# StanfordASL/pmpc

Measured on AMD Instinct MI355X. Metric: SCP iterations/sec (M particles x N horizon), higher is better.
Workload: dtype f64; 1 GPU; quadrotor x12 u4 M=4096 N=50 Nc=1 box-u, full SCP iteration (on-device linearise + c_lqp_solve-equivalent + residual), BASELINE config D; timed window = SCP iterations 6..2477 from the cold start X_prev = x0, U_prev = U_ref (the active-set round count falls as the SCP loop converges, so the rate depends on the window); particles_per_gpu=4096, parallelism=particle-shard x1, scp_loop=library (pmpc_scp_loop_device), ipm_warm_start=True

## Files before the change

include/pmpc_abi.h:

```cpp
#ifndef PMPC_ABI_H
#define PMPC_ABI_H

#include <stddef.h>

#ifdef __cplusplus
extern "C" {
#endif


void c_lqp_solve(double *X_out, double *U_out, size_t xdim, size_t udim, size_t N, size_t M, long long Nc,
                 double *x0, double *f, double *fx, double *fu, double *X_prev, double *U_prev, double *Q,
                 double *R, double *X_ref, double *U_ref, double *lx, double *ux, double *lu, double *uu,
                 double reg_x, double reg_u, double *slew_reg, double *slew_reg0, double *slew_um1,
                 long long verbose);

void c_lcone_solve(double *X_out, double *U_out, size_t xdim, size_t udim, size_t N, size_t M, long long Nc,
                   double *x0, double *f, double *fx, double *fu, double *X_prev, double *U_prev, double *Q,
                   double *R, double *X_ref, double *U_ref, double *lx, double *ux, double *lu, double *uu,
                   double reg_x, double reg_u, double *slew_reg, double *slew_reg0, double *slew_um1,
                   long long verbose, double smooth_alpha, char *solver);

void pmpc_lqp_solve_host(double *X_out, double *U_out, size_t xdim, size_t udim, size_t N, size_t M, long long Nc,
                         double *x0, double *f, double *fx, double *fu, double *X_prev, double *U_prev, double *Q,
                         double *R, double *X_ref, double *U_ref, double *lx, double *ux, double *lu, double *uu,
// ... 80 lines not shown
int pmpc_comm_unique_id(void *unique_id_128);
int pmpc_comm_init(pmpc_ctx *ctx, int rank, int world, const void *unique_id_128);
int pmpc_comm_init_mock(pmpc_ctx *ctx, int rank, int world, int group);
int pmpc_comm_rank(pmpc_ctx *ctx);
int pmpc_comm_world(pmpc_ctx *ctx);

int pmpc_linearize_device(pmpc_ctx *ctx, int model, size_t N, size_t M, const double *x0, const double *X_prev,
                          const double *U_prev, const double *params, double *f, double *fx, double *fu);

int pmpc_linearize_device_f32(pmpc_ctx *ctx, int model, size_t N, size_t M, const double *x0, const double *X_prev,
                              const double *U_prev, const double *params, double *f, float *fx, float *fu);

int pmpc_rollout_device(pmpc_ctx *ctx, int model, size_t N, size_t M, const double *x0, const double *U, const double *params, double *X);

int pmpc_shift_plan_device(pmpc_ctx *ctx, int model, size_t N, size_t M, size_t s, const double *X, const double *U,
                           const double *params, const double *U_tail, double *X_new, double *U_new, double *um1_new);

int pmpc_shift_active_set_device(pmpc_ctx *ctx, size_t N, size_t M, size_t udim, long long Nc, size_t s, const double *U,
                                 const double *U_tail, const int *act, const double *lo, const double *hi, double *U_new, int *act_new);

int pmpc_warm_shift_device(pmpc_ctx *ctx, size_t N, size_t M, size_t udim, long long Nc, size_t s, const double *U, const double *U_tail,
                           const double *lo, const double *hi, double *U_new, int *shifted);

int pmpc_warm_set_read_device(pmpc_ctx *ctx, int *act_out, size_t n);

int pmpc_linearize_compact_device(pmpc_ctx *ctx, int model, size_t N, size_t M, const double *x0, const double *X_prev,
                                  const double *U_prev, const double *params, double *f, double *jc);
int pmpc_expand_jac_device(pmpc_ctx *ctx, int model, size_t N, size_t M, const double *jc, double *fx, double *fu, int orient);
long long pmpc_jac_compact_doubles(int model, size_t N, size_t M);
int pmpc_jac_live_mask(int model, unsigned char *fx_mask, unsigned char *fu_mask);

int pmpc_as_sweep_variant(int sweep, int xdim, int udim, int M, int Nc, unsigned flags, const int *knobs, int *out);

int pmpc_as_sweep_launches(int sweep, unsigned long long *out, int n, int reset);
void pmpc_as_sweep_knobs(int *out);

int pmpc_scp_residual_device(pmpc_ctx *ctx, size_t xdim, size_t udim, size_t N, size_t M, const double *X, const double *X_prev,
                             const double *U, const double *U_prev, double *out);

int pmpc_scp_loop_device(pmpc_ctx *ctx, int model, const double *params, const pmpc_problem *p, double *f2, double *fx2, double *fu2,
                         int steps, int first_cold, double *res, pmpc_info *infos, int *last_in_out);

int pmpc_ref_shift_device(pmpc_ctx *ctx, size_t dim, size_t rows, const double *A, const double *c, const double *ref, double *out);
long long pmpc_ref_shift_bad_pivots(pmpc_ctx *ctx, int reset);

typedef struct pmpc_scp_cost {
  int kind;
  int K, pos_dim;
  int pos_idx[3];
  int per_stage;
  const double *centres, *sigma, *w;
} pmpc_scp_cost;
size_t pmpc_abi_scp_cost_size(void);

int pmpc_obstacle_cost_grad_device(pmpc_ctx *ctx, const pmpc_scp_cost *cost, size_t xdim, size_t N, size_t M, const double *X_prev,
                                   double *cx);
int pmpc_obstacle_ref_shift_device(pmpc_ctx *ctx, const pmpc_scp_cost *cost, size_t xdim, size_t N, size_t M, const double *X_prev,
                                   const double *Q, const double *X_ref, double *out);

int pmpc_scp_loop_device_cost(pmpc_ctx *ctx, int model, const double *params, const pmpc_problem *p, double *f2, double *fx2,
                              double *fu2, int steps, int first_cold, double *res, pmpc_info *infos, int *last_in_out,
                              const pmpc_scp_cost *cost);

typedef struct pmpc_scp_cstr {
  int kind;
  int K, pos_dim;
// ... 40 lines not shown
```

pmpc_amd/_lib.py:

```python
from __future__ import annotations

import ctypes
import os
from pathlib import Path

import numpy as np

_HERE = Path(__file__).resolve().parent
LIB_PATH = Path(os.environ["PMPC_HIP_LIB"]) if os.environ.get("PMPC_HIP_LIB") else _HERE / "libpmpc_hip.so"
_lib = None

c_dp = ctypes.POINTER(ctypes.c_double)

HAS_XBOUNDS, HAS_UBOUNDS, HAS_SLEW, HAS_SLEW0, FORCE_GENERIC, SYMMETRIC_COST, COLD_START, STATIC_CONS_BOUNDS, PREV_IS_LAST_SOLUTION, F32_MATRICES, CONE_OBJECTIVE = 1, 2, 4, 8, 16, 32, 64, 128, 256, 512, 1024

ABI_SYMBOLS = [
    "c_lqp_solve", "c_lcone_solve", "pmpc_lqp_solve_host", "pmpc_lcone_solve_host", "pmpc_create", "pmpc_destroy", "pmpc_stream", "pmpc_sync", "pmpc_lqp_solve_device",
    "pmpc_comm_unique_id", "pmpc_comm_init", "pmpc_comm_rank", "pmpc_comm_world", "pmpc_linearize_device",
    "pmpc_profile_enable", "pmpc_profile_read", "pmpc_version", "pmpc_lcone_solve_device", "pmpc_particle_costs_device", "pmpc_lsoc_solve_device", "pmpc_comm_init_mock",
    "pmpc_scp_residual_device", "pmpc_profile_read_partial", "pmpc_profile_read_all", "pmpc_scp_loop_device", "pmpc_linearize_device_f32",
    "pmpc_set_option", "pmpc_get_option", "pmpc_abi_struct_sizes", "pmpc_lcone_solve_host_ex", "pmpc_restart_stats",
    "pmpc_linearize_compact_device", "pmpc_expand_jac_device", "pmpc_jac_compact_doubles", "pmpc_jac_live_mask",
    "pmpc_as_sweep_variant", "pmpc_as_sweep_launches", "pmpc_as_sweep_knobs",
    "pmpc_ref_shift_device", "pmpc_ref_shift_bad_pivots", "pmpc_obstacle_cost_grad_device", "pmpc_obstacle_ref_shift_device",
    "pmpc_scp_loop_device_cost", "pmpc_abi_scp_cost_size",
    "pmpc_rollout_device", "pmpc_shift_plan_device",
    "pmpc_keepout_augment_device", "pmpc_abi_scp_cstr_size",
    "pmpc_keepout_strip_residual_device", "pmpc_scp_loop_device_cstr", "pmpc_abi_scp_aug_size", "pmpc_scp_loop_follow_ups",
    "pmpc_shift_active_set_device", "pmpc_warm_shift_device", "pmpc_warm_set_read_device",
]


class PmpcProblem(ctypes.Structure):
    _fields_ = (
        [(k, ctypes.c_size_t) for k in ("xdim", "udim", "N", "M")]
        + [("Nc", ctypes.c_longlong), ("flags", ctypes.c_uint), ("reg_x", ctypes.c_double), ("reg_u", ctypes.c_double)]
        + [(k, ctypes.c_void_p) for k in ("x0", "f", "fx", "fu", "X_prev", "U_prev", "Q", "R", "X_ref", "U_ref",
                                          "lx", "ux", "lu", "uu", "slew_reg", "slew_reg0", "slew_um1", "X_out", "U_out", "weights")]
        + [("barrier_mu", ctypes.c_double), ("soc_q", ctypes.c_size_t), ("soc_W", ctypes.c_void_p), ("soc_w0", ctypes.c_void_p),
           ("soc_v", ctypes.c_void_p), ("soc_v0", ctypes.c_double), ("soc_u_interior", ctypes.c_void_p),
           ("cone_count", ctypes.c_size_t), ("cone_sizes", ctypes.POINTER(ctypes.c_int)), ("cone_A", ctypes.c_void_p), ("cone_c", ctypes.c_void_p),
           ("cone_per_stage", ctypes.c_int), ("cone_k", ctypes.c_longlong), ("smooth_cstr", ctypes.c_int), ("smooth_beta", ctypes.c_double)]
    )


class PmpcInfo(ctypes.Structure):
    _fields_ = [("status", ctypes.c_int), ("ipm_iters", ctypes.c_int), ("structured_solves", ctypes.c_int),
                ("fast_path", ctypes.c_int), ("mu", ctypes.c_double), ("slack_res", ctypes.c_double),
                ("max_violation", ctypes.c_double), ("outer_solves", ctypes.c_int), ("active_set_rounds", ctypes.c_int)]


class PmpcScpCost(ctypes.Structure):
    _fields_ = [("kind", ctypes.c_int), ("K", ctypes.c_int), ("pos_dim", ctypes.c_int), ("pos_idx", ctypes.c_int * 3), ("per_stage", ctypes.c_int),
                ("centres", ctypes.c_void_p), ("sigma", ctypes.c_void_p), ("w", ctypes.c_void_p)]


# ... 50 lines not shown
    lib.pmpc_particle_costs_device.argtypes = [vp, ctypes.POINTER(PmpcProblem), vp, vp, vp]
    lib.pmpc_particle_costs_device.restype = ctypes.c_int
    lib.pmpc_comm_unique_id.argtypes = [vp]
    lib.pmpc_comm_unique_id.restype = ctypes.c_int
    lib.pmpc_comm_init.argtypes = [vp, ctypes.c_int, ctypes.c_int, vp]
    lib.pmpc_comm_init.restype = ctypes.c_int
    lib.pmpc_comm_init_mock.argtypes = [vp, ctypes.c_int, ctypes.c_int, ctypes.c_int]
    lib.pmpc_comm_init_mock.restype = ctypes.c_int
    lib.pmpc_comm_rank.argtypes = [vp]
    lib.pmpc_comm_rank.restype = ctypes.c_int
    lib.pmpc_comm_world.argtypes = [vp]
    lib.pmpc_comm_world.restype = ctypes.c_int
    lib.pmpc_linearize_device.argtypes = [vp, ctypes.c_int, sz, sz] + [vp] * 7
    lib.pmpc_linearize_device.restype = ctypes.c_int
    lib.pmpc_linearize_device_f32.argtypes = [vp, ctypes.c_int, sz, sz] + [vp] * 7
    lib.pmpc_linearize_device_f32.restype = ctypes.c_int
    if hasattr(lib, "pmpc_jac_live_mask"):
        lib.pmpc_linearize_compact_device.argtypes = [vp, ctypes.c_int, sz, sz] + [vp] * 6
        lib.pmpc_linearize_compact_device.restype = ctypes.c_int
        lib.pmpc_expand_jac_device.argtypes = [vp, ctypes.c_int, sz, sz, vp, vp, vp, ctypes.c_int]
        lib.pmpc_expand_jac_device.restype = ctypes.c_int
        lib.pmpc_jac_compact_doubles.argtypes = [ctypes.c_int, sz, sz]
        lib.pmpc_jac_compact_doubles.restype = ctypes.c_longlong
        lib.pmpc_jac_live_mask.argtypes = [ctypes.c_int, vp, vp]
        lib.pmpc_jac_live_mask.restype = ctypes.c_int
    if hasattr(lib, "pmpc_as_sweep_variant"):
        lib.pmpc_as_sweep_variant.argtypes = [ctypes.c_int] * 5 + [ctypes.c_uint, ctypes.POINTER(ctypes.c_int), ctypes.POINTER(ctypes.c_int)]
        lib.pmpc_as_sweep_variant.restype = ctypes.c_int
    if hasattr(lib, "pmpc_as_sweep_launches"):
        lib.pmpc_as_sweep_launches.argtypes = [ctypes.c_int, ctypes.POINTER(ctypes.c_ulonglong), ctypes.c_int, ctypes.c_int]
        lib.pmpc_as_sweep_launches.restype = ctypes.c_int
        lib.pmpc_as_sweep_knobs.argtypes = [ctypes.POINTER(ctypes.c_int)]
        lib.pmpc_as_sweep_knobs.restype = None
    lib.pmpc_scp_residual_device.argtypes = [vp, sz, sz, sz, sz] + [vp] * 5
    lib.pmpc_scp_residual_device.restype = ctypes.c_int
    lib.pmpc_profile_enable.argtypes = [vp, ctypes.c_int]
    lib.pmpc_profile_enable.restype = None
    lib.pmpc_profile_read.argtypes = [vp, c_dp, ctypes.POINTER(ctypes.c_longlong)]
    lib.pmpc_profile_read.restype = None
    lib.pmpc_profile_read_partial.argtypes = [vp, ctypes.POINTER(ctypes.c_double), ctypes.POINTER(ctypes.c_longlong)]
    lib.pmpc_profile_read_partial.restype = None
    lib.pmpc_restart_stats.argtypes = [vp, ctypes.POINTER(ctypes.c_ulonglong), ctypes.c_int]
    lib.pmpc_restart_stats.restype = None
    lib.pmpc_profile_read_all.argtypes = [vp, c_dp, ctypes.POINTER(ctypes.c_longlong), ctypes.c_int]
    lib.pmpc_profile_read_all.restype = None
    lib.pmpc_scp_loop_device.argtypes = [vp, ctypes.c_int, vp, ctypes.POINTER(PmpcProblem), vp, vp, vp, ctypes.c_int, ctypes.c_int, vp,
                                         ctypes.POINTER(PmpcInfo), ctypes.POINTER(ctypes.c_int)]
    lib.pmpc_scp_loop_device.restype = ctypes.c_int
    if hasattr(lib, "pmpc_scp_loop_device_cost"):
        lib.pmpc_ref_shift_device.argtypes = [vp, sz, sz, vp, vp, vp, vp]
        lib.pmpc_ref_shift_device.restype = ctypes.c_int
        lib.pmpc_ref_shift_bad_pivots.argtypes = [vp, ctypes.c_int]
        lib.pmpc_ref_shift_bad_pivots.restype = ctypes.c_longlong
        lib.pmpc_obstacle_cost_grad_device.argtypes = [vp, ctypes.POINTER(PmpcScpCost), sz, sz, sz, vp, vp]
        lib.pmpc_obstacle_cost_grad_device.restype = ctypes.c_int
        lib.pmpc_obstacle_ref_shift_device.argtypes = [vp, ctypes.POINTER(PmpcScpCost), sz, sz, sz, vp, vp, vp, vp]
        lib.pmpc_obstacle_ref_shift_device.restype = ctypes.c_int
        lib.pmpc_scp_loop_device_cost.argtypes = lib.pmpc_scp_loop_device.argtypes + [ctypes.POINTER(PmpcScpCost)]
        lib.pmpc_scp_loop_device_cost.restype = ctypes.c_int
        lib.pmpc_abi_scp_cost_size.argtypes = []
        lib.pmpc_abi_scp_cost_size.restype = sz
        if lib.pmpc_abi_scp_cost_size() != ctypes.sizeof(PmpcScpCost):
            raise ImportError(f"{LIB_PATH} and pmpc_amd/_lib.py disagree on pmpc_scp_cost: library {lib.pmpc_abi_scp_cost_size()} bytes, "
                              f"binding {ctypes.sizeof(PmpcScpCost)}: rebuild the library")
    if hasattr(lib, "pmpc_shift_plan_device"):
        lib.pmpc_rollout_device.argtypes = [vp, ctypes.c_int, sz, sz, vp, vp, vp, vp]
# ... 36 lines not shown
    sp, si = sz(0), sz(0)
    lib.pmpc_abi_struct_sizes(ctypes.byref(sp), ctypes.byref(si))
    if (sp.value, si.value) != (ctypes.sizeof(PmpcProblem), ctypes.sizeof(PmpcInfo)):
        raise ImportError(f"{LIB_PATH} ({lib.pmpc_version().decode()}) and pmpc_amd/_lib.py disagree on the ABI structs: library "
                          f"{sp.value}/{si.value} bytes, binding {ctypes.sizeof(PmpcProblem)}/{ctypes.sizeof(PmpcInfo)}: rebuild the library")
    _lib = lib
    return lib


def jac_live_mask(model: int, x: int, u: int):
    lib = load()
    mx, mu = np.zeros(x * x, dtype=np.uint8), np.zeros(x * u, dtype=np.uint8)
    got = lib.pmpc_jac_live_mask(int(model), mx.ctypes.data, mu.ctypes.data)
    if got < 0:
        raise ValueError(f"model {model} is not a built-in model")
    if got != 100 * x + u:
        raise ValueError(f"model {model}: compact records are for dims {got // 100} x {got % 100}, not {x} x {u}")
    return mx.reshape(x, x).T.astype(bool), mu.reshape(u, x).T.astype(bool)


AS_SWEEP_FLAGS = ("defect", "as_settled_in", "mat32", "cone_H", "xb_D", "as_uraw", "as_T")


def as_sweep_variant(sweep: str, x: int, u: int, M: int, Nc: int, flags: int, knobs=None):
    lib = load()
    out = (ctypes.c_int * 8)()
    kn = (ctypes.c_int * 3)(*knobs) if knobs is not None else None
    got = lib.pmpc_as_sweep_variant({"bwd": 0, "fwd": 1}[sweep], x, u, M, Nc, flags, kn, out)
    if got < 0:
        raise ValueError(f"({x}, {u}) is not a compiled pair of the active-set sweeps")
    return tuple(out[:5]), bool(got), tuple(bool(v) for v in out[5:8])


def as_sweep_code(sweep: str, variant) -> int:
    a, b, c, d, e = (int(v) for v in variant)
    if sweep == "bwd":
        return a + 3 * (b + 2 * (c + 2 * (d + 3 * e)))
    return a + 2 * b + 4 * c + 8 * d + 16 * e


def as_sweep_launches(sweep: str, reset: bool = False):
    lib = load()
    sw = {"bwd": 0, "fwd": 1}[sweep]
    n = lib.pmpc_as_sweep_launches(sw, None, 0, 0)
    out = (ctypes.c_ulonglong * n)()
    lib.pmpc_as_sweep_launches(sw, out, n, int(reset))
    return [int(v) for v in out]


def scp_loop_follow_ups(reset: bool = False):
    out = (ctypes.c_ulonglong * 2)()
    load().pmpc_scp_loop_follow_ups(out, int(reset))
    return int(out[0]), int(out[1])


def as_sweep_knobs():
    out = (ctypes.c_int * 3)()
    load().pmpc_as_sweep_knobs(out)
    return tuple(out)


def dptr(a: np.ndarray):
    assert a.dtype == np.float64 and a.flags["C_CONTIGUOUS"]
    return a.ctypes.data_as(c_dp)
```

pmpc_amd/csrc/fast_common.h:

```cpp
#pragma once
#include "pmpc_dev.h"

namespace {

typedef double v4d __attribute__((ext_vector_type(4)));

__device__ __forceinline__ v4d mfma(double a, double b, v4d c) {
  return __builtin_amdgcn_mfma_f64_16x16x4f64(a, b, c, 0, 0, 0);
}
__device__ __forceinline__ double readlane_d(double v, int l) {
  int lo = __builtin_amdgcn_readlane(__double2loint(v), l);
  int hi = __builtin_amdgcn_readlane(__double2hiint(v), l);
  return __hiloint2double(hi, lo);
}
__device__ __forceinline__ double rfl_d(double v) {
  int lo = __builtin_amdgcn_readfirstlane(__double2loint(v));
  int hi = __builtin_amdgcn_readfirstlane(__double2hiint(v));
  return __hiloint2double(hi, lo);
}
template <int CTRL>
__device__ __forceinline__ double dpp_d(double v) {
  int lo = __builtin_amdgcn_mov_dpp(__double2loint(v), CTRL, 0xF, 0xF, true);
  int hi = __builtin_amdgcn_mov_dpp(__double2hiint(v), CTRL, 0xF, 0xF, true);
  return __hiloint2double(hi, lo);
}
__device__ __forceinline__ double row_allsum(double v) {
  v += dpp_d<0xB1>(v);
  v += dpp_d<0x4E>(v);
  v += dpp_d<0x141>(v);
  v += dpp_d<0x140>(v);
  return v;
}
__device__ __forceinline__ void swap32_d(double v, double &a, double &b) {
  auto lo = __builtin_amdgcn_permlane32_swap(__double2loint(v), __double2loint(v), false, false);
  auto hi = __builtin_amdgcn_permlane32_swap(__double2hiint(v), __double2hiint(v), false, false);
  a = __hiloint2double(hi[0], lo[0]);
  b = __hiloint2double(hi[1], lo[1]);
}
__device__ __forceinline__ void swap16_d(double v, double &a, double &b) {
  auto lo = __builtin_amdgcn_permlane16_swap(__double2loint(v), __double2loint(v), false, false);
  auto hi = __builtin_amdgcn_permlane16_swap(__double2hiint(v), __double2hiint(v), false, false);
  a = __hiloint2double(hi[0], lo[0]);
  b = __hiloint2double(hi[1], lo[1]);
}
__device__ __forceinline__ double grp_allsum(double v) {
  double a, b;
  swap32_d(v, a, b);
  v = a + b;
  swap16_d(v, a, b);
  return a + b;
}
__device__ __forceinline__ void grp_gather(double v, double (&out)[4]) {
  double p01, p23;
  swap32_d(v, p01, p23);
  swap16_d(p01, out[0], out[1]);
  swap16_d(p23, out[2], out[3]);
}
__device__ __forceinline__ double rsqrt_d(double d) {
  const double r = __builtin_amdgcn_rsq(d);
  const double e = fma(-0.5 * d * r, r, 0.5);
  return fma(r, e, r);
}
__device__ __forceinline__ const double *badd(const double *p, long long bytes) {
  return (const double *)((const char *)p + bytes);
// ... 103 lines not shown
```

pmpc_amd/csrc/kernels_as.hip:

```cpp
#include <atomic>
#include <type_traits>

#include "fast_common.h"
#include "as_ctl_dev.h"
#include "as_variant.h"
#include "../../include/pmpc_abi.h"
#include "jac_compact.h"

#ifdef PMPC_STAGE_TIMELINE
#define PMPC_TL_STAMPS 10
__device__ unsigned long long pmpc_tl[3][128][PMPC_TL_STAMPS];
#define TL_DECL(kind) unsigned long long tl_[PMPC_TL_STAMPS] = {}; const int tl_kind = (kind); const bool tl_on = blockIdx.x == gridDim.x / 2
#define TL(k) do { __builtin_amdgcn_sched_barrier(0); tl_[k] = __builtin_amdgcn_s_memtime(); __builtin_amdgcn_sched_barrier(0); } while (0)
#define TL_FLUSH(j) do { if (tl_on && threadIdx.x == 0 && (j) < 128) { for (int k_ = 0; k_ < PMPC_TL_STAMPS; k_++) pmpc_tl[tl_kind][j][k_] = tl_[k_]; } } while (0)
#else
#define TL_DECL(kind)
#define TL(k)
#define TL_FLUSH(j)
#endif

#ifndef PMPC_AS_LEAN_WAVES
#define PMPC_AS_LEAN_WAVES 4
#endif
#ifndef PMPC_AS_DEEP_WAVES
#define PMPC_AS_DEEP_WAVES 3
#endif
#ifndef PMPC_AS_DEEP2_MAXM
#define PMPC_AS_DEEP2_MAXM 1024
#endif

namespace {

template <int XD, int UD, int MODE, bool SKIP, bool DEFECT, int EX = 0, class MT = double>
__global__ void __launch_bounds__(64, MODE == 2 ? 2 : (MODE == 1 ? PMPC_AS_DEEP_WAVES : PMPC_AS_LEAN_WAVES)) k_bwd_as(LQArgs a) {
  constexpr bool CONE = EX == 1, XBOX = EX == 2;
  typedef Lane<XD, UD> LT;
  constexpr int KS = LT::KS, XP = LT::XP;
  constexpr bool PADX = (XD != XP);
  constexpr long long D8 = sizeof(double);
  constexpr bool DEEP = MODE != 0, SCHOL = !DEEP;
  constexpr long long MB = sizeof(MT);
  if (a.done && *a.done) return;
  const int lane = threadIdx.x;
  const int N = a.N, Nc = a.Nc, i = a.as_perm ? __builtin_amdgcn_readfirstlane(a.as_perm[blockIdx.x]) : (int)blockIdx.x;
  if (SKIP && a.as_settled_in[i]) {
    const int nc = Nc * UD;
    if (lane < nc) {
      const double *H = a.Hc_part + (size_t)i * nc * nc;
      double acc = 0.0;
      for (int cc = 0; cc < nc; cc++) acc = fma(H[(lane < cc ? lane : cc) + nc * (lane < cc ? cc : lane)], a.as_delta[cc], acc);
      a.gc_part[(size_t)i * nc + lane] += acc;
    }
    return;
  }
  const LT L(lane);
  const int g = L.g, c = L.c;
  const size_t pbase = (size_t)i * N;
  const bool own0 = (i == 0 && a.owner);
  const bool gu = g < UD;
  const double *Z = a.zeros;
  const double pwt = a.pw ? a.pw[i] : 1.0;
  const double regx = pwt * a.reg_x, regu = pwt * a.reg_u;
  const double *Xb = DEFECT ? a.X_prev : a.Xb, *Ub = DEFECT ? a.U_prev : a.Ub;
  constexpr int CKS = 64 * KS + 32;
  int jtop = N - 1, ck_k = 0;
  if (SKIP && a.as_ck) {
    const int jh = a.as_jhi[i];
// ... 5 lines not shown
      atomicAdd(a.ck_stat + (ck_k ? 1 : 3), (unsigned long long)(jtop + 1));
    }
  }
  const double *ck_ = a.as_ck ? ubase(a.as_ck, (long long)i * a.ck_slots * (long long)(CKS * sizeof(double))) : nullptr;

  const bool fF = L.cxv || L.cu;
  const MT *pF = L.cxv ? (const MT *)a.fx + (pbase + jtop) * (XD * XD) + XD * L.oc + L.row0
                       : (L.cu ? (const MT *)a.fu + (pbase + jtop) * (XD * UD) + XD * L.cb + L.row0 : (const MT *)Z);
  int sF = fF ? -(int)MB * (L.cxv ? XD * XD : XD * UD) : 0;
  typedef typename jacc::SpecFor<XD, UD>::list JSpecs;
  if constexpr (JSpecs::COUNT > 0 && std::is_same<MT, double>::value) {
    if (a.jac_compact) {
      const jacc::LaneSel js = jacc::select(JSpecs{}, a.jac_compact, lane);
      const int m = js.bwd;
      if (m != jacc::NONE) {
        pF = m >= 0 ? (const MT *)a.fx + (pbase + jtop) * js.rec + m : (const MT *)a.fx + (size_t)a.M * N * js.rec + (size_t)i * js.pool + (-1 - m);
        sF = m >= 0 ? -(int)MB * js.rec : 0;
      }
    }
  }
  const unsigned lQ = (unsigned)((L.cxv ? XD * L.oc + L.row0 : 0) * MB);
  const double pwt_x = L.cxv ? pwt : 0.0;
  const bool fR = L.cu && gu;
  const unsigned lR = (unsigned)((fR ? g + UD * L.cb : 0) * MB), lRd = (unsigned)((fR ? g + UD * L.cb : 0) * D8);
  const unsigned lxr = (unsigned)(L.row0 * D8), lxc = (unsigned)((L.cxv ? L.oc : 0) * D8);
  const unsigned lug = (unsigned)((gu ? g : 0) * D8);
  const double regx_c = L.cxv ? regx : 0.0;
  const bool umask = L.cu && g == L.cb;
  const double umask_d = umask ? 1.0 : 0.0;
  const bool diag_x = L.cxv && ((c & 3) == g);
  bool dmask[KS];
#pragma unroll
  for (int r = 0; r < KS; r++) dmask[r] = diag_x && (c >> 2) == r;
  const long long px = (long long)(pbase * XD) * D8, pu = (long long)(pbase * UD) * D8;
  const double *Xb_ = ubase(Xb, px), *Xr_ = ubase(a.X_ref, px), *Xp_ = ubase(a.X_prev, px), *f_ = ubase(a.f, px);
  const double *kff_ = ubase(a.kff, pu);
  const void *Q_ = ubase_v(a.Q, (long long)(pbase * (XD * XD)) * MB), *R_ = ubase_v(a.R, (long long)(pbase * (UD * UD)) * MB);
  const void *K_ = ubase_v(a.K, (long long)(pbase * 64) * MB);
  auto xoff = [&](int jj) { return (long long)(jj * (int)(XD * D8)); };
  auto uoff = [&](int jj) { return (long long)(jj * (int)(UD * D8)); };
  auto ld_Q = [&](int jj, double *dst) {
    const void *q = ubase_v(Q_, (long long)(jj * (int)(XD * XD * MB)));
#pragma unroll
    for (int r = 0; r < KS; r++) {
      const bool rv = !PADX || (L.row0 + r < XD);
      const double v = ldom<MT>(q, rv ? lQ + r * (unsigned)MB : 0u);
      dst[r] = rv ? v : 0.0;
    }
  };
  auto ld_xm = [&](int jj, double *dst) {
    const double *xb = ubase(Xb_, xoff(jj)), *xr = ubase(Xr_, xoff(jj));
#pragma unroll
    for (int r = 0; r < KS; r++) {
      const bool rv = !PADX || (L.row0 + r < XD);
      const unsigned o = rv ? lxr + r * 8u : 0u;
      const double v = pwt * (ldo(xb, o) - ldo(xr, o));
      dst[r] = rv ? v : 0.0;
    }
  };
  auto ld_gx = [&](int jj) -> double {
    if (DEFECT) return 0.0;
    return regx_c * (ldo(ubase(Xb_, xoff(jj)), lxc) - ldo(ubase(Xp_, xoff(jj)), lxc));
  };
  const char *pC = (const char *)Z;
  int sC = 0;
  if (gu && c == XP) { pC = (const char *)(Ub + (pbase + jtop) * UD + g); sC = -UD * (int)D8; }
// ... 104 lines not shown
    for (int r = 0; r < KS; r++) Fr[r] = (!MAIN && j == 0 && L.cxv) ? 0.0 : cur.F[r];
    const double Rc = cur.R;
    const double um_g = pwt * (dpp_d<0x00>(cur.ctl) - dpp_d<0x55>(cur.ctl));
    const int act_g = __builtin_amdgcn_mov_dpp(__double2loint(cur.ctl), 0xAA, 0xF, 0xF, true);
    Du_c = (umask && act_g) ? a.as_big : 0.0;
    const double gu_c0 = DEFECT ? 0.0 : regu_s * dpp_d<0x140>(cur.ctl);
    const bool cone_here = CONE && (MAIN || !cons || own0);
    double gu_c = gu_c0;
    if constexpr (CONE) gu_c = fma(dpp_d<0xFF>(cur.ctl), cone_here ? umask_d : 0.0, gu_c0);
    double Hcone = 0.0;
    if constexpr (CONE) Hcone = cone_here ? cur.ch : 0.0;
    const double df_c = (DEFECT && L.cxv) ? cur.f - xb_carry : 0.0;
    if (DEFECT) xb_carry = cur.xb;
    gx_c = DEFECT ? 0.0 : regx_c * (cur.xb - cur.xp);
    if constexpr (XBOX) gx_c += cur.xg;
    col_to_row<KS>(pwt_x * (cur.xb - cur.xr), g, xm_row);
#pragma unroll
    for (int r = 0; r < KS; r++) Qc[r] = cur.Q[r];
    auto late_pf = [&]() { if (below) fetch_late(j - 1, j >= 2 ? j - 2 : 0, nxt); };
    TL(1);
    if (MODE == 1) late_pf();
    if (MODE != 2 && below) fetch_early(j - 1, nxt);
    TL(2);

    if (DEFECT) {
#pragma unroll
      for (int r = 0; r < KS; r++) s_row[r] += row_allsum(S[r] * df_c);
    }
    double hp = fma(Rc, um_g, gu_c);
#pragma unroll
    for (int r = 0; r < KS; r++) hp = fma(Fr[r], s_row[r], hp);
    const double h_col = grp_allsum(hp);
    double hu[UD];
#pragma unroll
    for (int b = 0; b < UD; b++) hu[b] = readlane_d(h_col, XP + b);

    TL(3);
    v4d H = {0.0, 0.0, 0.0, 0.0};
    double p2q = 0.0;
    if (below) {
#pragma unroll
      for (int r = 0; r < KS; r++) {
        if constexpr (XBOX) H[r] = fma(pwt_x, Qc[r], dmask[r] ? regx + cur.xd : 0.0);
        else H[r] = fma(pwt_x, Qc[r], dmask[r] ? regx : 0.0);
        p2q = fma(Qc[r], xm_row[r], p2q);
      }
    }
    if constexpr (CONE) H[KS] = fma(pwt, Rc, (umask ? regu : 0.0) + (cons ? 0.0 : Du_c + Hcone));
    else H[KS] = fma(pwt, Rc, (umask ? regu : 0.0) + (cons ? 0.0 : Du_c));
    v4d G = {0.0, 0.0, 0.0, 0.0};
#pragma unroll
    for (int r = 0; r < KS; r++) G = mfma(S[r], Fr[r], G);
#pragma unroll
    for (int r = 0; r < KS; r++) H = mfma(Fr[r], G[r], H);

    if (!DEEP && !MAIN) late_pf();
    if (!MAIN && cons) {
      double v = H[KS];
      if (own0) v += CONE ? Du_c + Hcone : Du_c;
      const int nc = Nc * UD;
      if (L.cu && gu) a.Hc_part[(size_t)i * nc * nc + (size_t)(j * UD + g) + (size_t)nc * (j * UD + L.cb)] = v;
      st_rec(j, (L.cxv && gu) ? H[KS] : 0.0);
#pragma unroll
      for (int r = 0; r < KS; r++) S[r] = H[r];
      if (lane < UD) a.gc_part[(size_t)i * (Nc * UD) + j * UD + lane] = pick<UD>(hu, lane);
      if (j == 0) return;
      const double p2 = grp_allsum(p2q);
      s_col = L.cxv ? h_col + p2 + gx_c : 0.0;
      col_to_row<KS>(s_col, g, s_row);
      return;
    }

    TL(4);
    double Lc[UD][UD], Ld[UD], col[UD];
#pragma unroll
    for (int q = 0; q < UD; q++) {
#pragma unroll
      for (int pp = q; pp < UD; pp++) {
        double v = readlane_d(H[KS], (XP + q) + 16 * pp);
#pragma unroll
        for (int k = 0; k < q; k++) v -= Lc[pp][k] * Lc[q][k];
        if (pp == q) {
          bad |= !(v > 0.0);
          Ld[q] = SCHOL ? rfl_d(rsqrt_d(v)) : rsqrt_d(v);
        } else {
          Lc[pp][q] = SCHOL ? rfl_d(v * Ld[q]) : v * Ld[q];
        }
      }
    }
    TL(5);
    double rows4[4];
    grp_gather(H[KS], rows4);
#pragma unroll
    for (int k = 0; k < UD; k++) col[k] = L.cu ? (L.cb == k ? 1.0 : 0.0) : rows4[k];
    chol_solve<UD>(Lc, Ld, col);
    const double Kg = pick<UD>(col, g);
    const double rec = frec ? Kg : 0.0;
    TL(6);
    v4d Sn = mfma(H[KS], (L.cxv && gu) ? -Kg : 0.0, H);
#pragma unroll
    for (int r = 0; r < KS; r++) S[r] = Sn[r];
    st_rec(j, rec);
    if (!DEEP && MAIN) {
      __builtin_amdgcn_sched_barrier(0);
      late_pf();
    }
    const double Kreg = L.cxv ? rec : 0.0;
    const double hug = pick<UD>(hu, g);
    double kq = L.cu ? rec * pick<UD>(hu, L.cb) : 0.0;
    kq += dpp_d<0xB1>(kq);
    kq += dpp_d<0x4E>(kq);
    if (c == XP && gu) gsto(ubase(kff_, uoff(j)), lug, kq);
    TL(7);
    if (!MAIN && j == 0) { TL_FLUSH(j); return; }
    const double red2 = grp_allsum(fma(-Kreg, hug, p2q));
    s_col = L.cxv ? h_col + red2 + gx_c : 0.0;
    col_to_row<KS>(s_col, g, s_row);
    TL(8);
    TL_FLUSH(j);
  };

  const int jmin = Nc > 1 ? Nc : 1;
  int j = jtop;
  if (MODE == 2) {
    Pipe P0, P1, P2;
    auto fetch = [&](int jj, Pipe &q) {
      const int k = jj > 0 ? jj : 0;
      fetch_early(k, q);
      fetch_late(k, k >= 1 ? k - 1 : 0, q);
    };
    fetch(jtop, P0);
    fetch(jtop - 1, P1);
    for (; j - 2 >= jmin; j -= 3) {
      fetch(j - 2, P2);
      stage(std::true_type{}, j, P0, P0);
      __builtin_amdgcn_sched_barrier(0);
      fetch(j - 3, P0);
      stage(std::true_type{}, j - 1, P1, P1);
      __builtin_amdgcn_sched_barrier(0);
      fetch(j - 4, P1);
      stage(std::true_type{}, j - 2, P2, P2);
      __builtin_amdgcn_sched_barrier(0);
    }
    for (; j >= 0; j--) {
      fetch(j - 2, P2);
      if (j >= jmin) stage(std::true_type{}, j, P0, P0);
      else stage(std::false_type{}, j, P0, P0);
      P0 = P1;
      P1 = P2;
    }
  } else {
    Pipe A, B;
    fetch_early(jtop, A);
    fetch_late(jtop, jtop >= 1 ? jtop - 1 : 0, A);
    for (; j >= jmin; j--) {
      stage(std::true_type{}, j, A, B);
      A = B;
    }
    if (j >= jmin) {
      stage(std::true_type{}, j, A, B);
      A = B;
      j--;
    }
    for (; j >= 0; j--) {
      stage(std::false_type{}, j, A, B);
      A = B;
    }
  }
  if (bad && lane == 0) *a.fail = 2;
}

template <int XD, int UD, bool DEFECT, bool PF2, bool CONE = false, class MT = double, bool SENS = false>
__global__ void __launch_bounds__(64, 4) k_fwd_as(LQArgs a) {
  typedef Lane<XD, UD> LT;
  constexpr int KS = LT::KS;
  constexpr bool PADX = (XD != LT::XP);
  constexpr long long D8 = sizeof(double);
  if (a.done && *a.done) return;
  const int lane = threadIdx.x;
  const LT L(lane);
  const int N = a.N, Nc = a.Nc, i = a.as_perm ? __builtin_amdgcn_readfirstlane(a.as_perm[blockIdx.x]) : (int)blockIdx.x, g = L.g, c = L.c;
  const size_t pbase = (size_t)i * N;
  const bool gu = g < UD;
  const double *Z = a.zeros;
  constexpr int MB = (int)sizeof(MT);
  const char *pA = (const char *)Z, *pB = (const char *)Z;
  int sAr = 0, sAj = 0, sBj = 0;
// ... 212 lines not shown
    pS += UD * (int)D8;
    if (store_u) gsto_i(ubase(act_, uoff(j) >> 1), lug >> 1, anew);
    TL(4);
    D[KS] = 0.0;
    double bop = (c < 4 && gu) ? du_q : 0.0;
    if (SENS) {
      const bool sc = c >= 4 && c < 4 + UD && gu;
      const double bs = (!MAIN && j < Nc) ? ((g == c - 4) ? 1.0 : 0.0) : -raw;
      bop = sc ? bs : bop;
    }
    D = mfma(cur.T[KS], bop, D);
    if (SENS) {
      if (c >= 4 && c < 4 + UD) {
        typedef double v2dd __attribute__((ext_vector_type(2)));
        const v2dd lo2 = {D[0], KS > 1 ? D[KS > 1 ? 1 : 0] : 0.0}, hi2 = {KS > 2 ? D[KS > 2 ? 2 : 0] : 0.0, gu ? bop : 0.0};
        __attribute__((address_space(1))) char *t = (__attribute__((address_space(1))) char *)(unsigned long long)ubase(T_, (long long)(j * (int)(64 * D8))) + lT;
        *(v2dd __attribute__((address_space(1))) *)t = lo2;
        *(v2dd __attribute__((address_space(1))) *)(t + 16) = hi2;
      }
    }
    if (DEFECT) {
      const double dfo = own_x ? cur.f - cur.xb : 0.0;
      D[0] += dpp_d<0x00>(dfo);
      if (KS > 1) D[1] += dpp_d<0x55>(dfo);
      if (KS > 2) D[2] += dpp_d<0xAA>(dfo);
    }
    if (own_x) {
      double mine = D[0];
#pragma unroll
      for (int r = 1; r < KS; r++) mine = (c == r) ? D[r] : mine;
      gsto(ubase(Xo_, xoff(j)), lx1, cur.xb + mine);
    }
#pragma unroll
    for (int r = 0; r < KS; r++) V[r] = (c < (SENS ? 4 + UD : 4)) ? D[r] : 0.0;
    TL(5);
    TL_FLUSH(j);
  };

  int nrel_e = 0, nadd_e = 0, nbad_e = 0, jh_e = -1;
  auto settled_update = [&](int j0) {
    double dl[UD];
#pragma unroll
    for (int k = 0; k < UD; k++) dl[k] = readlane_d(dcap, 16 * k);
    const int s16 = lane & 15, q4 = lane >> 4, gs = s16 >> 2, rs = s16 & 3;
    const bool is_x = rs < KS && KS * gs + rs < XD, is_u = rs == 3 && gs < UD;
    const size_t xo = (size_t)(is_x ? KS * gs + rs : 0), uo = (size_t)(is_u ? gs : 0);
    constexpr int SB = 4;
    for (int j4 = j0; j4 < N; j4 += 4 * SB) {
      double dv[SB], xv[SB], ub[SB], kf[SB], lo[SB], hi[SB];
      int act[SB];
#pragma unroll
      for (int q = 0; q < SB; q++) {
        const int jj = j4 + 4 * q + q4, jc = jj < N ? jj : N - 1;
        const double *t = a.as_T + (pbase + jc) * 64 + s16;
        double acc = 0.0;
#pragma unroll
        for (int k = 0; k < UD; k++) acc = fma(gld(t + 16 * k), dl[k], acc);
        dv[q] = acc;
        xv[q] = is_x ? gld(Xb + (pbase + jc) * XD + xo) : 0.0;
        const size_t e = (pbase + jc) * UD + uo;
        ub[q] = is_u ? gld(Ub + e) : 0.0;
        kf[q] = is_u ? gld(a.kff + e) : 0.0;
        lo[q] = is_u ? gld(a.as_lo + e) : 0.0;
        hi[q] = is_u ? gld(a.as_hi + e) : 0.0;
        act[q] = is_u ? a.as_act[e] : 0;
      }
#pragma unroll
// ... 177 lines not shown
  if (!launched) no_such_variant("forward sweep of an active-set round", XD, UD);
}

}

#ifdef PMPC_STAGE_TIMELINE
extern "C" int pmpc_debug_timeline_read(unsigned long long *out) {
  return (int)hipMemcpyFromSymbol(out, HIP_SYMBOL(pmpc_tl), sizeof(unsigned long long) * 3 * 128 * PMPC_TL_STAMPS);
}
#endif
static bool as_dims_compiled(int x, int u) {
#define X(xd, ud) if (x == xd && u == ud) return true;
  PMPC_FAST_DIMS(X)
#undef X
  return false;
}
bool f32_as_dims_supported(int x, int u) { return as_dims_compiled(x, u) && as_f32_dims(x, u); }
bool xbox_as_dims_supported(int x, int u) { return as_dims_compiled(x, u) && as_xbox_dims(x, u); }
bool cone_as_dims_supported(int x, int u) { return as_dims_compiled(x, u) && as_cone_dims(x, u); }
int pmpc_as_sweep_variant(int sweep, int xdim, int udim, int M, int Nc, unsigned flags, const int *knobs, int *out) {
  if ((sweep != 0 && sweep != 1) || !as_dims_compiled(xdim, udim) || !out) return -1;
  const AsSweepKnobs k = knobs ? AsSweepKnobs{knobs[0], knobs[1], knobs[2]} : AsSweepKnobs{PMPC_AS_DEEP2_MAXM, PMPC_AS_DEEP_WAVES * 1024, 1 << 30};
  const bool defect = flags & 1, settled_in = flags & 2, mat32 = flags & 4, cone_H = flags & 8, xb_D = flags & 16, as_uraw = flags & 32, as_T = flags & 64;
  out[5] = f32_as_dims_supported(xdim, udim); out[6] = cone_as_dims_supported(xdim, udim); out[7] = xbox_as_dims_supported(xdim, udim);
  if (sweep == 0) {
    const BwdAsVariant v = select_bwd_as(M, defect, settled_in, mat32, cone_H, xb_D, k);
    out[0] = v.mode; out[1] = v.skip; out[2] = v.defect; out[3] = v.ex; out[4] = v.f32;
    return bwd_as_compiled(v, xdim, udim);
  }
  const FwdAsVariant v = select_fwd_as(M, Nc, defect, mat32, as_uraw, as_T, k);
  out[0] = v.defect; out[1] = v.pf2; out[2] = v.cone; out[3] = v.f32; out[4] = v.sens;
  return fwd_as_compiled(v, xdim, udim);
}
int pmpc_as_sweep_launches(int sweep, unsigned long long *out, int n, int reset) {
  if (sweep != 0 && sweep != 1) return -1;
  std::atomic<unsigned long long> *t = sweep == 0 ? as_bwd_launches : as_fwd_launches;
  const int codes = sweep == 0 ? AS_BWD_CODES : AS_FWD_CODES;
  for (int c = 0; c < codes; c++) {
    const unsigned long long v = reset ? t[c].exchange(0, std::memory_order_relaxed) : t[c].load(std::memory_order_relaxed);
    if (out && c < n) out[c] = v;
  }
  return codes;
}
void pmpc_as_sweep_knobs(int *out) {
  const AsSweepKnobs &k = as_sweep_knobs();
  out[0] = k.deep2_maxm; out[1] = k.deep_maxm; out[2] = k.fwd_pf2_maxm;
}
void launch_bwd_as(const LQArgs &a, hipStream_t s) {
#define X(xd, ud) if (a.x == xd && a.u == ud) { launch_bwd_as_t<xd, ud>(a, s); return; }
  PMPC_FAST_DIMS(X)
#undef X
  no_such_variant("factor sweep of an active-set round", a.x, a.u);
}
void launch_fwd_as(const LQArgs &a, hipStream_t s) {
#define X(xd, ud) if (a.x == xd && a.u == ud) { launch_fwd_as_t<xd, ud>(a, s); return; }
  PMPC_FAST_DIMS(X)
#undef X
  no_such_variant("forward sweep of an active-set round", a.x, a.u);
}
void launch_as_ctl(AsCtl *ctl, const int *cnt_part, int M, const int *fail, int reduce, int decide, int last_of_batch, AsCtl *mirror,
                   unsigned long long *mirror_seq, unsigned long long seq, hipStream_t s, double *tail, const double *viol, const int *open_part) {
  hipLaunchKernelGGL(k_as_ctl, dim3(1), dim3(1024), 0, s, ctl, cnt_part, M, fail, reduce, decide, last_of_batch, mirror, mirror_seq, seq, tail, viol,
                     open_part);
}
void launch_as_perm(const int *settled, int M, int *perm, const int *done, hipStream_t s) {
  hipLaunchKernelGGL(k_as_perm, dim3(1), dim3(1024), 0, s, settled, M, perm, done);
// ... 5 lines not shown
```

Before: 3017 SCP iterations/s.

## Tighten backward active-set sweep registers to fit four waves for x12u4

```diff
diff --git a/include/pmpc_abi.h b/include/pmpc_abi.h
--- a/include/pmpc_abi.h
+++ b/include/pmpc_abi.h
@@ -136,6 +136,8 @@
 
 int pmpc_as_sweep_variant(int sweep, int xdim, int udim, int M, int Nc, unsigned flags, const int *knobs, int *out);
 
+int pmpc_as_sweep_resources(int sweep, int xdim, int udim, const int *variant, int *out);
+
 int pmpc_as_sweep_launches(int sweep, unsigned long long *out, int n, int reset);
 void pmpc_as_sweep_knobs(int *out);
 
diff --git a/pmpc_amd/_lib.py b/pmpc_amd/_lib.py
--- a/pmpc_amd/_lib.py
+++ b/pmpc_amd/_lib.py
@@ -21,7 +21,7 @@
     "pmpc_scp_residual_device", "pmpc_profile_read_partial", "pmpc_profile_read_all", "pmpc_scp_loop_device", "pmpc_linearize_device_f32",
     "pmpc_set_option", "pmpc_get_option", "pmpc_abi_struct_sizes", "pmpc_lcone_solve_host_ex", "pmpc_restart_stats",
     "pmpc_linearize_compact_device", "pmpc_expand_jac_device", "pmpc_jac_compact_doubles", "pmpc_jac_live_mask",
-    "pmpc_as_sweep_variant", "pmpc_as_sweep_launches", "pmpc_as_sweep_knobs",
+    "pmpc_as_sweep_variant", "pmpc_as_sweep_launches", "pmpc_as_sweep_knobs", "pmpc_as_sweep_resources",
     "pmpc_ref_shift_device", "pmpc_ref_shift_bad_pivots", "pmpc_obstacle_cost_grad_device", "pmpc_obstacle_ref_shift_device",
     "pmpc_scp_loop_device_cost", "pmpc_abi_scp_cost_size",
     "pmpc_rollout_device", "pmpc_shift_plan_device",
@@ -138,6 +138,9 @@
         lib.pmpc_as_sweep_launches.restype = ctypes.c_int
         lib.pmpc_as_sweep_knobs.argtypes = [ctypes.POINTER(ctypes.c_int)]
         lib.pmpc_as_sweep_knobs.restype = None
+    if hasattr(lib, "pmpc_as_sweep_resources"):
+        lib.pmpc_as_sweep_resources.argtypes = [ctypes.c_int] * 3 + [ctypes.POINTER(ctypes.c_int), ctypes.POINTER(ctypes.c_int)]
+        lib.pmpc_as_sweep_resources.restype = ctypes.c_int
     lib.pmpc_scp_residual_device.argtypes = [vp, sz, sz, sz, sz] + [vp] * 5
     lib.pmpc_scp_residual_device.restype = ctypes.c_int
     lib.pmpc_profile_enable.argtypes = [vp, ctypes.c_int]
@@ -240,6 +243,18 @@
     return tuple(out[:5]), bool(got), tuple(bool(v) for v in out[5:8])
 
 
+def as_sweep_resources(sweep: str, x: int, u: int, variant):
+    out = (ctypes.c_int * 4)()
+    got = load().pmpc_as_sweep_resources({"bwd": 0, "fwd": 1}[sweep], x, u, (ctypes.c_int * 5)(*(int(v) for v in variant)), out)
+    if got == -2:
+        return None
+    if got == -1:
+        raise ValueError(f"({x}, {u}) is not a compiled pair of the active-set sweeps")
+    if got != 0:
+        raise RuntimeError(f"pmpc_as_sweep_resources: HIP error {got}")
+    return dict(zip(("regs", "scratch_bytes", "lds_bytes", "max_threads"), (int(v) for v in out)))
+
+
 def as_sweep_code(sweep: str, variant) -> int:
     a, b, c, d, e = (int(v) for v in variant)
     if sweep == "bwd":
diff --git a/pmpc_amd/csrc/fast_common.h b/pmpc_amd/csrc/fast_common.h
--- a/pmpc_amd/csrc/fast_common.h
+++ b/pmpc_amd/csrc/fast_common.h
@@ -30,6 +30,15 @@
   v += dpp_d<0x141>(v);
   v += dpp_d<0x140>(v);
   return v;
+}
+template <int C0, int NB>
+__device__ __forceinline__ double row_own_bcast(double v) {
+  static_assert(NB >= 1 && NB <= 4 && C0 >= 0 && C0 + NB <= 16, "row_own_bcast: lanes C0 .. C0 + NB - 1 of a 16-lane row");
+  double o = NB == 4 ? __builtin_amdgcn_update_dpp(0.0, v, 0x150 + C0, 0xF, 0xF, true) : __builtin_amdgcn_update_dpp(0.0, v, 0x150 + C0, 0x1, 0xF, false);
+  if (NB > 1) o = __builtin_amdgcn_update_dpp(o, v, 0x150 + C0 + (NB > 1 ? 1 : 0), 0x2, 0xF, false);
+  if (NB > 2) o = __builtin_amdgcn_update_dpp(o, v, 0x150 + C0 + (NB > 2 ? 2 : 0), 0x4, 0xF, false);
+  if (NB > 3) o = __builtin_amdgcn_update_dpp(o, v, 0x150 + C0 + (NB > 3 ? 3 : 0), 0x8, 0xF, false);
+  return o;
 }
 __device__ __forceinline__ void swap32_d(double v, double &a, double &b) {
   auto lo = __builtin_amdgcn_permlane32_swap(__double2loint(v), __double2loint(v), false, false);
diff --git a/pmpc_amd/csrc/kernels_as.hip b/pmpc_amd/csrc/kernels_as.hip
--- a/pmpc_amd/csrc/kernels_as.hip
+++ b/pmpc_amd/csrc/kernels_as.hip
@@ -31,8 +31,9 @@
 
 namespace {
 
+#define AS_DEEP_FITS4 (XD == 12 && UD == 4 && DEFECT && !SKIP && EX == 0 && sizeof(MT) == 8)
 template <int XD, int UD, int MODE, bool SKIP, bool DEFECT, int EX = 0, class MT = double>
-__global__ void __launch_bounds__(64, MODE == 2 ? 2 : (MODE == 1 ? PMPC_AS_DEEP_WAVES : PMPC_AS_LEAN_WAVES)) k_bwd_as(LQArgs a) {
+__global__ void __launch_bounds__(64, MODE == 2 ? 2 : (MODE == 1 ? (AS_DEEP_FITS4 ? 4 : PMPC_AS_DEEP_WAVES) : PMPC_AS_LEAN_WAVES)) k_bwd_as(LQArgs a) {
   constexpr bool CONE = EX == 1, XBOX = EX == 2;
   typedef Lane<XD, UD> LT;
   constexpr int KS = LT::KS, XP = LT::XP;
@@ -104,6 +105,9 @@
   bool dmask[KS];
 #pragma unroll
   for (int r = 0; r < KS; r++) dmask[r] = diag_x && (c >> 2) == r;
+  int unit_hi[UD];
+#pragma unroll
+  for (int k = 0; k < UD; k++) unit_hi[k] = L.cb == k ? 0x3FF00000 : 0;
   const long long px = (long long)(pbase * XD) * D8, pu = (long long)(pbase * UD) * D8;
   const double *Xb_ = ubase(Xb, px), *Xr_ = ubase(a.X_ref, px), *Xp_ = ubase(a.X_prev, px), *f_ = ubase(a.f, px);
   const double *kff_ = ubase(a.kff, pu);
@@ -274,8 +278,10 @@
     for (int r = 0; r < KS; r++) hp = fma(Fr[r], s_row[r], hp);
     const double h_col = grp_allsum(hp);
     double hu[UD];
-#pragma unroll
-    for (int b = 0; b < UD; b++) hu[b] = readlane_d(h_col, XP + b);
+    if constexpr (!MAIN) {
+#pragma unroll
+      for (int b = 0; b < UD; b++) hu[b] = readlane_d(h_col, XP + b);
+    }
 
     TL(3);
     v4d H = {0.0, 0.0, 0.0, 0.0};
@@ -334,7 +340,8 @@
     double rows4[4];
     grp_gather(H[KS], rows4);
 #pragma unroll
-    for (int k = 0; k < UD; k++) col[k] = L.cu ? (L.cb == k ? 1.0 : 0.0) : rows4[k];
+    for (int k = 0; k < UD; k++)
+      col[k] = __hiloint2double(c < XP ? __double2hiint(rows4[k]) : unit_hi[k], c < XP ? __double2loint(rows4[k]) : 0);
     chol_solve<UD>(Lc, Ld, col);
     const double Kg = pick<UD>(col, g);
     const double rec = frec ? Kg : 0.0;
@@ -348,8 +355,10 @@
       late_pf();
     }
     const double Kreg = L.cxv ? rec : 0.0;
-    const double hug = pick<UD>(hu, g);
-    double kq = L.cu ? rec * pick<UD>(hu, L.cb) : 0.0;
+    double hug, huc;
+    if constexpr (MAIN) { hug = row_own_bcast<XP, UD>(h_col); huc = h_col; }
+    else { hug = pick<UD>(hu, g); huc = pick<UD>(hu, L.cb); }
+    double kq = L.cu ? rec * huc : 0.0;
     kq += dpp_d<0xB1>(kq);
     kq += dpp_d<0x4E>(kq);
     if (c == XP && gu) gsto(ubase(kff_, uoff(j)), lug, kq);
@@ -395,6 +404,12 @@
     Pipe A, B;
     fetch_early(jtop, A);
     fetch_late(jtop, jtop >= 1 ? jtop - 1 : 0, A);
+    if constexpr (AS_DEEP_FITS4) {
+      for (; j - 1 >= jmin; j -= 2) {
+        stage(std::true_type{}, j, A, B);
+        stage(std::true_type{}, j - 1, B, A);
+      }
+    }
     for (; j >= jmin; j--) {
       stage(std::true_type{}, j, A, B);
       A = B;
@@ -673,7 +688,7 @@
       gsto(ubase(Xo_, xoff(j)), lx1, cur.xb + mine);
     }
 #pragma unroll
-    for (int r = 0; r < KS; r++) V[r] = (c < (SENS ? 4 + UD : 4)) ? D[r] : 0.0;
+    for (int r = 0; r < KS; r++) V[r] = D[r];
     TL(5);
     TL_FLUSH(j);
   };
@@ -917,6 +932,36 @@
   out[0] = v.defect; out[1] = v.pf2; out[2] = v.cone; out[3] = v.f32; out[4] = v.sens;
   return fwd_as_compiled(v, xdim, udim);
 }
+namespace {
+template <int XD, int UD>
+int as_sweep_attr_t(int sweep, const int *f, hipFuncAttributes *attr) {
+  int got = -2;
+  if (sweep == 0) {
+    if (f[0] < 0 || f[0] > 2 || f[3] < 0 || f[3] > 2) return -2;
+    lift3(f[0], [&](auto MODE) { lift(f[1] != 0, [&](auto SKIP) { lift(f[2] != 0, [&](auto DEFECT) { lift3(f[3], [&](auto EX) { lift(f[4] != 0, [&](auto F32) {
+      if constexpr (bwd_as_compiled(BwdAsVariant{MODE, SKIP, DEFECT, EX, F32}, XD, UD))
+        got = (int)hipFuncGetAttributes(attr, (const void *)&k_bwd_as<XD, UD, MODE, SKIP, DEFECT, EX, std::conditional_t<F32, float, double>>);
+    }); }); }); }); });
+  } else {
+    lift(f[0] != 0, [&](auto DEFECT) { lift(f[1] != 0, [&](auto PF2) { lift(f[2] != 0, [&](auto CONE) { lift(f[3] != 0, [&](auto F32) { lift(f[4] != 0, [&](auto SENS) {
+      if constexpr (fwd_as_compiled(FwdAsVariant{DEFECT, PF2, CONE, F32, SENS}, XD, UD))
+        got = (int)hipFuncGetAttributes(attr, (const void *)&k_fwd_as<XD, UD, DEFECT, PF2, CONE, std::conditional_t<F32, float, double>, SENS>);
+    }); }); }); }); });
+  }
+  return got;
+}
+}
+int pmpc_as_sweep_resources(int sweep, int xdim, int udim, const int *variant, int *out) {
+  if ((sweep != 0 && sweep != 1) || !as_dims_compiled(xdim, udim) || !variant || !out) return -1;
+  hipFuncAttributes attr = {};
+  int got = -1;
+#define X(xd, ud) if (xdim == xd && udim == ud) got = as_sweep_attr_t<xd, ud>(sweep, variant, &attr);
+  PMPC_FAST_DIMS(X)
+#undef X
+  if (got != 0) return got;
+  out[0] = attr.numRegs; out[1] = (int)attr.localSizeBytes; out[2] = (int)attr.sharedSizeBytes; out[3] = attr.maxThreadsPerBlock;
+  return 0;
+}
 int pmpc_as_sweep_launches(int sweep, unsigned long long *out, int n, int reset) {
   if (sweep != 0 && sweep != 1) return -1;
   std::atomic<unsigned long long> *t = sweep == 0 ? as_bwd_launches : as_fwd_launches;
```

Result: faster. 3126 SCP iterations/s, median of 6 (+3.6%).
